# davidbau/rewriting

Measured on AMD Instinct MI355X. Metric: images/sec StyleGANv2-1024 fwd, higher is better.
Workload: dtype f32 (conv operands split into exact f16 pairs from 32x32 up, f32 accumulate); 1 GPU; stylegan2-1024 generator forward (FFHQ-1024 architecture); batch_per_gpu=64, mconv=seq, weights=synthetic seed 0, parallelism=seeds partitioned per rank, no collective, matrix_mode=split, direct_sums=auto

## Files before the change

rewriting_amd/csrc/rw_common.h:

```cpp
#pragma once
#include <hip/hip_runtime.h>
#include <stdint.h>
#include <stdlib.h>
#include "../../include/rewriting_hip.h"

#define RW_WAVE 64

#define RW_CHECK_ARG(cond) do { if (!(cond)) return RW_ERR_BAD_ARGUMENT; } while (0)
#define RW_LAUNCH_RESULT() ((int)hipGetLastError())

static inline hipStream_t rw_s(rw_stream_t s) { return (hipStream_t)s; }

static inline int64_t rw_cdiv(int64_t a, int64_t b) { return (a + b - 1) / b; }

static inline int rw_cu_count(void) {
  static int cached[64];
  int dev = 0;
  if (hipGetDevice(&dev) != hipSuccess || dev < 0 || dev >= 64) return 256;
  if (cached[dev] == 0) {
    int n = 0;
    cached[dev] = (hipDeviceGetAttribute(&n, hipDeviceAttributeMultiprocessorCount, dev) == hipSuccess && n > 0) ? n : 256;
  }
  return cached[dev];
}
// ... 104 lines not shown
    ib += g_ib + carry;
  }
};

__device__ __forceinline__ int rw_swz(int cc) { return (cc >> 1) & 3; }
__device__ __forceinline__ rw_f16x8 rw_expand(rw_f32x2 w) {
  const rw_f32x4 d = {w[0], w[1], w[0], w[1]};
  return __builtin_bit_cast(rw_f16x8, d);
}
__device__ __forceinline__ rw_f16x8 rw_pair(rw_f16x8 a, rw_f16x8 b) {
  return rw_f16x8{a[0], a[1], a[2], a[3], b[0], b[1], b[2], b[3]};
}
__device__ __forceinline__ rw_f16x8 rw_pair(rw_f32x2 a, rw_f32x2 b) {
  const rw_f32x4 d = {a[0], a[1], b[0], b[1]};
  return __builtin_bit_cast(rw_f16x8, d);
}
__device__ __forceinline__ rw_f16x8 rw_split4(float v0, float v1, float v2, float v3) {
  const rw_f16x2 h01 = __builtin_convertvector(rw_f32x2{v0, v1}, rw_f16x2);
  const rw_f16x2 h23 = __builtin_convertvector(rw_f32x2{v2, v3}, rw_f16x2);
  float r0, r1, r2, r3;
  asm("v_fma_mix_f32 %0, -%1, 1.0, %2 op_sel_hi:[1,0,0]" : "=v"(r0) : "v"(h01), "v"(v0));
  asm("v_fma_mix_f32 %0, -%1, 1.0, %2 op_sel:[1,0,0] op_sel_hi:[1,0,0]" : "=v"(r1) : "v"(h01), "v"(v1));
  asm("v_fma_mix_f32 %0, -%1, 1.0, %2 op_sel_hi:[1,0,0]" : "=v"(r2) : "v"(h23), "v"(v2));
  asm("v_fma_mix_f32 %0, -%1, 1.0, %2 op_sel:[1,0,0] op_sel_hi:[1,0,0]" : "=v"(r3) : "v"(h23), "v"(v3));
  const rw_f16x2 l01 = __builtin_convertvector(rw_f32x2{r0, r1}, rw_f16x2);
  const rw_f16x2 l23 = __builtin_convertvector(rw_f32x2{r2, r3}, rw_f16x2);
  return rw_f16x8{h01[0], h01[1], h23[0], h23[1], l01[0], l01[1], l23[0], l23[1]};
}

__device__ __forceinline__ void rw_dma_buffer_b32(unsigned lds_addr, int voffset, rw_i32x4 rsrc, int soffset) {
  asm volatile("s_mov_b32 m0, %0\n\ts_nop 0\n\tbuffer_load_dword %1, %2, %3 offen lds"
               :: "s"(lds_addr), "v"(voffset), "s"(rsrc), "s"(soffset) : "memory");
}
__device__ __forceinline__ void rw_dma_global_b32(unsigned lds_addr, const void* gptr) {
  asm volatile("s_mov_b32 m0, %0\n\ts_nop 0\n\tglobal_load_lds_dword %1, off" :: "s"(lds_addr), "v"(gptr) : "memory");
}
__device__ __forceinline__ void rw_dma_global_b128_s(unsigned lds_addr, int voffset, const void* sbase) {
  asm volatile("s_mov_b32 m0, %0\n\ts_nop 0\n\tglobal_load_lds_dwordx4 %1, %2" :: "s"(lds_addr), "v"(voffset), "s"(sbase)
               : "memory");
}

__device__ __forceinline__ void rw_lds_barrier() {
  asm volatile("" ::: "memory");
  __builtin_amdgcn_s_waitcnt(0xC07F);
  __builtin_amdgcn_s_barrier();
  asm volatile("" ::: "memory");
}

__device__ __forceinline__ __amdgpu_buffer_rsrc_t rw_image_rsrc(const float* x, int ib, int in_ch, int64_t hw) {
  return __builtin_amdgcn_make_buffer_rsrc(const_cast<float*>(x + (int64_t)ib * in_ch * hw), 0,
                                           (int)((int64_t)in_ch * hw * 4), 0x00020000);
}

static inline int64_t rw_bound_slot_capacity(int64_t n_elems) { return 2048 + n_elems / 1024 + 1; }

int rw_bound_finish(float* bound, int64_t nslots, hipStream_t stream);

__device__ __forceinline__ float rw_bound_load(const float* __restrict__ bound) {
  return rw_wave_max(bound[threadIdx.x & 63]);
}

__device__ __forceinline__ void rw_bound_store_wave(float* __restrict__ bound, float v) {
  if ((threadIdx.x & 63) == 0)
    bound[RW_BOUND_LANES + (int64_t)blockIdx.x * (blockDim.x >> 6) + (threadIdx.x >> 6)] = v;
}

// ... 72 lines not shown
```

rewriting_amd/csrc/rw_wino4.hip:

```cpp
#include "rw_common.h"

#ifndef W4_ABL
#define W4_ABL 0
#endif
#ifndef W4_SETPRIO
#define W4_SETPRIO 0
#endif

__host__ __device__ constexpr int w4_nat(int pos) { return pos < 18 ? pos : (pos < 26 ? pos + 10 : pos - 8); }

struct Wino4Problem {
  const float* x; const float* uf; float* y;
  const float* style; const float* demod; const float* noise; const float* noise_w; const float* bias;
  int batch, in_ch, out_ch, h, w;
  int groups_x, groups_y, gpw;
  float w_scale;
  int act;
  const float* rgb_weight; const float* rgb_style; const float* rgb_bias; const float* rgb_skip; float* rgb_out;
  float rgb_scale;
  const float* post;
  const float* x_amax; float* y_amax;
  float u_inv;
};

// ... 208 lines not shown
  };

  fetch(0, 0);
  uload(0, 0);
  uload(1, 1 % NC);
  stash(0);
  fetch(1 / NC, 1 % NC);
  __syncthreads();

  int c = 0, g = 0, ub = 0;
  int fg = 2 / NC, fc = 2 % NC;
  for (int v = 0; v < VT; ++v) {
    const int buf = v & 1;
    const int ub2 = ub == 0 ? 2 : ub - 1;
    if (!(W4_ABL & 2)) {
      stash(buf ^ 1);
      fetch(fg, fc);
    }
    if (!(W4_ABL & 4)) uload(ub2, c + 2 < NC ? c + 2 : c + 2 - NC);
    compute(buf, ub);
    if (c == NC - 1) {
      if (!(W4_ABL & 8) || acc[0][0] == 12345.f) group_epilogue(g);
      c = 0; ++g;
    } else { ++c; }
    if (++fc == NC) { fc = 0; ++fg; }
    ub = ub == 2 ? 0 : ub + 1;
    if (!(W4_ABL & 16)) {
      __builtin_amdgcn_s_waitcnt(0xC07F);
      __builtin_amdgcn_s_barrier();
    }
  }
}

#define W4B_PITCH 68
#ifndef W4_NTS
#define W4_NTS 0
#endif
#if W4_NTS
#define W4_STORE(ptr, val) __builtin_nontemporal_store((val), reinterpret_cast<rw_f32x4*>(ptr))
#else
#define W4_STORE(ptr, val) (*reinterpret_cast<rw_f32x4*>(ptr) = (val))
#endif
#ifndef W4C_PREFETCH
#define W4C_PREFETCH 0
#endif

__device__ __forceinline__ void w4_bt2_rows(const rw_f32x2 e0, const rw_f32x2 e2, const rw_f32x2 e4, const rw_f32x2 d1,
                                            const rw_f32x2 d2, const rw_f32x2 d3, const rw_f32x2 d4, float cA, float cB,
                                            float cC, rw_f32x2& o0, rw_f32x2& o1, rw_f32x2& o2) {
  o0 = 4.f * e0 - 5.f * e2 + e4;
  const rw_f32x2 p = d4 - cA * d2, q = cB * d3 - cC * d1;
  o1 = p + q; o2 = p - q;
}
__device__ __forceinline__ void w4_at_row(const float (&t)[6], float (&v)[4]) {
  const float s1 = t[1] + t[2], s2 = t[1] - t[2], s3 = t[3] + t[4], s4 = t[3] - t[4];
  v[0] = t[0] + s1 + s3; v[1] = s2 + 2.f * s4; v[2] = s1 + 4.f * s3; v[3] = s2 + 8.f * s4 + t[5];
}

__device__ __forceinline__ void w4_split16(float v, rw_f16x2& hh, rw_f16x2& ll) {
  if (W4_ABL & 32) { hh = __builtin_bit_cast(rw_f16x2, v); ll = hh; return; }
  hh = __builtin_convertvector(rw_f32x2{v, v}, rw_f16x2);
  float r;
  asm("v_fma_mix_f32 %0, -%1, 1.0, %2 op_sel_hi:[1,0,0]" : "=v"(r) : "v"(hh), "v"(v));
  ll = __builtin_convertvector(rw_f32x2{r, r}, rw_f16x2);
}
__device__ __forceinline__ rw_f32x4 w4_mfma16(rw_u32x2 ww, rw_f16x2 hh, rw_f16x2 ll, rw_f32x4 acc) {
  const rw_f16x4 a = __builtin_bit_cast(rw_f16x4, ww);
  const rw_f16x4 b = {hh[0], hh[1], ll[0], ll[1]};
  if (W4_ABL & 64) {
    asm volatile("" :: "v"(a), "v"(b));
    return acc;
  }
  return __builtin_amdgcn_mfma_f32_16x16x16f16(a, b, acc, 0, 0, 0);
}
__device__ __forceinline__ unsigned w4_pack16(float u) {
  const _Float16 h = (_Float16)u;
  const _Float16 l = (_Float16)(u - (float)h);
  return (unsigned)__builtin_bit_cast(unsigned short, h) | ((unsigned)__builtin_bit_cast(unsigned short, l) << 16);
}

template <int WGN, int UDEPTH, int MODE, bool STYLE, bool PS = false, bool H16 = false>
__device__ __forceinline__ void conv_wino36b_body(const Wino4Problem& p) {
  static_assert(!PS || (WGN == 2 && UDEPTH == 2), "the point split is written for the <2, 2> shape");
  constexpr bool UP = MODE == 1, RGB = MODE == 2;
  constexpr int NSZ = RGB ? 384 : (UP ? 512 : 256);
  constexpr int NST = RGB ? 3 : 16;
  constexpr int WGM = 2;
  constexpr int WAVES = WGM * WGN, THREADS = 64 * WAVES;
  constexpr int PR = 4 * WGN + 2;
  constexpr int PIECES = (PR * W4B_PITCH + 63) / 64;
  constexpr int PPW = 4 * PIECES / WAVES;
  static_assert(4 * PIECES % WAVES == 0, "patch pieces divide among the waves");
  constexpr int UPW = (9 * WGM + WAVES - 1) / WAVES;
  constexpr int PSZ = 4 * PIECES * 64;
  constexpr int USZ = WGM * 9 * 256;
  __shared__ __attribute__((aligned(16))) float Ps[3 * PSZ];
  __shared__ __attribute__((aligned(16))) float Us[UDEPTH * USZ];
  __shared__ __attribute__((aligned(16))) float Ns[WAVES * NSZ];
  __shared__ float St[512];
  __shared__ float Ct[2][16 * WGM];
  __shared__ float Cr[3][16 * WGM];
  __shared__ float Red[WAVES];

  const int tid = threadIdx.x, lane = tid & 63;
  const int wave = __builtin_amdgcn_readfirstlane(tid >> 6);
  const int wm = wave / WGN, wn = wave % WGN;
  const int lk = lane >> 4, lt = lane & 15;

  const int local = rw_xcd_remap(blockIdx.x, gridDim.x);
  const int o_tiles = p.out_ch / (16 * WGM);
  const int runs_x = p.groups_x / p.gpw;
  const int ot = local % o_tiles;
  int pg = local / o_tiles;
  const int run = pg % runs_x; pg /= runs_x;
  const int gy = pg % p.groups_y;
  const int ib = pg / p.groups_y;
  const int o0 = ot * 16 * WGM;
  const int y0 = gy * 4 * WGN, gx0 = run * p.gpw;
  const int64_t hw = (int64_t)p.h * p.w;
  const float* xb = p.x + (int64_t)ib * p.in_ch * hw;
  const int NC = p.in_ch >> 2;
  const int VT = p.gpw * NC;

  float in_scale = 1.f, out_scale = 1.f;
  if (H16) {
    float smax = p.style ? 0.f : 1.f;
    if (p.style)
      for (int i = tid; i < p.in_ch; i += THREADS) smax = fmaxf(smax, fabsf(p.style[(int64_t)ib * p.in_ch + i]));
#pragma unroll
    for (int off = 32; off; off >>= 1) smax = fmaxf(smax, __shfl_xor(smax, off));
    smax = rw_block_max<WAVES>(smax, lane, wave, Red);
    rw_split_scales<8>(rw_bound_load(p.x_amax) * smax, p.u_inv, in_scale, out_scale);
  }
  for (int i = tid; i < p.in_ch; i += THREADS) St[i] = (p.style ? p.style[(int64_t)ib * p.in_ch + i] : 1.0f) * in_scale;
  if (tid < 16 * WGM) {
    const int o = UP ? (o0 + tid) >> 2 : o0 + tid;
    const int real_ch = UP ? p.out_ch >> 2 : p.out_ch;
    Ct[0][tid] = (p.demod ? p.demod[(int64_t)ib * real_ch + o] * p.w_scale : p.w_scale) * out_scale;
    Ct[1][tid] = p.act ? p.bias[o] : 0.f;
    if (RGB) {
      const float sr = p.rgb_scale * p.rgb_style[(int64_t)ib * p.out_ch + o];
#pragma unroll
      for (int cc = 0; cc < 3; ++cc) Cr[cc][tid] = sr * p.rgb_weight[cc * p.out_ch + o];
    }
  }
  const float noise_w = p.noise ? p.noise_w[0] : 0.f;

  typedef __attribute__((address_space(3))) float* lds_f;
  const unsigned ps_base = (unsigned)(size_t)(lds_f)Ps, us_base = (unsigned)(size_t)(lds_f)Us,
                 ns_base = (unsigned)(size_t)(lds_f)Ns;
  const unsigned long long xaddr = (unsigned long long)xb;
  const rw_i32x4 xsrc = {(int)(unsigned)xaddr, (int)(unsigned)(xaddr >> 32), (int)((int64_t)p.in_ch * hw * 4),
                         0x00020000};
  const int hw4 = (int)hw * 4;
  static_assert(PIECES % PPW == 0, "a wave's pieces lie in one channel");
  const int pch = (wave * PPW) / PIECES, piece0 = (wave * PPW) % PIECES;
  int xoff[PPW];
  auto set_group = [&](int g) __attribute__((always_inline)) {
    const int x0 = (gx0 + g) * 64;
#pragma unroll
    for (int s = 0; s < PPW; ++s) {
      const int f = 64 * (piece0 + s) + lane;
      const int r = f / W4B_PITCH, c = f - r * W4B_PITCH;
      const int iy = y0 - 1 + r, ix = x0 - 1 + c;
      const bool ok = r < PR && c < W4_PC && iy >= 0 && iy < p.h && ix >= 0 && ix < p.w;
      xoff[s] = ok ? (iy * p.w + ix) * 4 : 0x7fffffff;
    }
  };
  int p_soff = 0;
  unsigned p_dst = 0;
  auto pload_begin = [&](int ring, int fg, int fc) __attribute__((always_inline)) {
    if (fc == 0) set_group(fg);
    p_soff = (4 * fc + pch) * hw4;
    p_dst = ps_base + (unsigned)((ring * PSZ + pch * (PIECES * 64) + 64 * piece0) * 4);
  };
  auto pload_piece = [&](int s) __attribute__((always_inline)) { rw_dma_buffer_b32(p_dst + 256 * s, xoff[s], xsrc, p_soff); };
  auto pload = [&](int ring, int fg, int fc) __attribute__((always_inline)) {
    pload_begin(ring, fg, fc);
#pragma unroll
    for (int s = 0; s < PPW; ++s) pload_piece(s);
  };
  const int kq_total = p.in_ch >> 2;
  const int a_lane = lane * 4;
  auto uload = [&](int ring, int kq) __attribute__((always_inline)) {
#pragma unroll
    for (int t = 0; t < UPW; ++t) {
      const int j = wave + WAVES * t;
      if (j < 9 * WGM) {
        const int ob = j / 9, q = j - 9 * ob;
        const float* src = p.uf + ((int64_t)((o0 >> 4) + ob) * kq_total + kq) * (9 * 256) + q * 256;
        rw_dma_global_b128_s(us_base + (unsigned)((ring * USZ + ob * (9 * 256) + q * 256) * 4), a_lane * 4, src);
      }
    }
  };
  auto nload = [&](int g) __attribute__((always_inline)) {
    if (UP) {
      const float* sb = p.noise + (int64_t)ib * 4 * hw + (int64_t)(2 * (y0 + 4 * wn) + 4 * wm) * (2 * p.w)
                        + (gx0 + g) * 128;
      const int vo = ((lane >> 5) * (2 * p.w) + 4 * (lane & 31)) * 4;
#pragma unroll
      for (int j = 0; j < 2; ++j)
        rw_dma_global_b128_s(ns_base + (unsigned)((wn * 1024 + (4 * wm + 2 * j) * 128) * 4), vo,
                             sb + (int64_t)(2 * j) * (2 * p.w));
      return;
    }
    const float* np = p.noise + (int64_t)ib * hw + (int64_t)(y0 + 4 * wn) * p.w + (gx0 + g) * 64 + lane;
#pragma unroll
    for (int r = 0; r < 4; ++r) rw_dma_global_b32(ns_base + (unsigned)((wave * NSZ + 64 * r) * 4), np + (int64_t)r * p.w);
  };

  rw_f32x4 acc[36];
#pragma unroll
  for (int xi = 0; xi < 36; ++xi) acc[xi] = rw_f32x4{0.f, 0.f, 0.f, 0.f};
  float ymax = 0.f;

  const int item_off = lk * (PIECES * 64) + (4 * wn) * W4B_PITCH + 4 * lt;
  auto compute = [&](int ring, int uring, int kq, auto spread_tag) __attribute__((always_inline)) {
    constexpr bool SPREAD = decltype(spread_tag)::value != 0;
    const float* base = &Us[uring * USZ + wm * (9 * 256) + a_lane];
    const float* src = &Ps[ring * PSZ + item_off];
    const float sv = St[4 * kq + lk];
    rw_f32x4 a4[3];
    a4[0] = *reinterpret_cast<const rw_f32x4*>(base);
    a4[1] = *reinterpret_cast<const rw_f32x4*>(base + 256);
    a4[2] = *reinterpret_cast<const rw_f32x4*>(base + 512);
    rw_f32x2 c2[6][3];
#pragma unroll
    for (int r = 0; r < 6; ++r) {
      const rw_f32x4 lo = *reinterpret_cast<const rw_f32x4*>(src + r * W4B_PITCH);
      if (STYLE) {
        c2[r][0] = rw_f32x2{lo[0], lo[1]} * sv;
        c2[r][1] = rw_f32x2{lo[2], lo[3]} * sv;
        c2[r][2] = *reinterpret_cast<const rw_f32x2*>(src + r * W4B_PITCH + 4) * sv;
      } else {
        c2[r][0] = rw_f32x2{lo[0], lo[1]};
        c2[r][1] = rw_f32x2{lo[2], lo[3]};
        c2[r][2] = *reinterpret_cast<const rw_f32x2*>(src + r * W4B_PITCH + 4);
      }
    }
    float d[6][6];
#pragma unroll
    for (int cp = 0; cp < 3; ++cp)
      if (!(W4_ABL & 1)) w4_bt2(c2[0][cp], c2[1][cp], c2[2][cp], c2[3][cp], c2[4][cp], c2[5][cp]);
#pragma unroll
    for (int a = 0; a < 6; ++a) {
      if (!(W4_ABL & 1)) {
        w4_bt_row(c2[a][0], c2[a][1], c2[a][2], d[a]);
      } else {
        d[a][0] = c2[a][0][0]; d[a][1] = c2[a][0][1]; d[a][2] = c2[a][1][0]; d[a][3] = c2[a][1][1];
        d[a][4] = c2[a][2][0]; d[a][5] = c2[a][2][1];
      }
    }
#if W4_SETPRIO
    __builtin_amdgcn_s_setprio(W4_SETPRIO);
#endif
#pragma unroll
    for (int q = 0; q < 9; ++q) {
      const rw_f32x4 a = a4[q % 3];
      if (q + 3 < 9) a4[q % 3] = *reinterpret_cast<const rw_f32x4*>(base + (q + 3) * 256);
      if (SPREAD && !(W4_ABL & 2)) {
        if (2 * q < PPW) pload_piece(2 * q);
        if (2 * q + 1 < PPW) pload_piece(2 * q + 1);
      }
      __builtin_amdgcn_sched_barrier(0);
#pragma unroll
      for (int e = 0; e < 4; ++e) {
        const int xi = w4_nat(4 * q + e);
        acc[xi] = __builtin_amdgcn_mfma_f32_16x16x4f32(a[e], d[xi / 6][xi % 6], acc[xi], 0, 0, 0);
      }
    }
#if W4_SETPRIO
    __builtin_amdgcn_s_setprio(0);
#endif
  };

  auto aread = [&](unsigned addr, auto pos_tag, rw_u32x2& dst) __attribute__((always_inline)) {
    constexpr int POS = decltype(pos_tag)::value;
    if (W4_ABL & 128) { dst = rw_u32x2{addr, (unsigned)POS}; return; }
    asm volatile("ds_read2st64_b32 %0, %1 offset0:%2 offset1:%2" : "=&v"(dst) : "v"(addr), "n"(POS));
  };
  auto compute16 = [&](int ring, int uring, int kq, auto spread_tag) __attribute__((always_inline)) {
    constexpr bool SPREAD = decltype(spread_tag)::value != 0;
    const unsigned ua = us_base + (unsigned)((uring * USZ + wm * (9 * 256) + lane) * 4);
    const float* src = &Ps[ring * PSZ + item_off];
    const float sv = St[4 * kq + lk];
    rw_f32x2 c2[6][3];
#pragma unroll
    for (int r = 0; r < 6; ++r) {
      const rw_f32x4 lo = *reinterpret_cast<const rw_f32x4*>(src + r * W4B_PITCH);
      c2[r][0] = rw_f32x2{lo[0], lo[1]} * sv;
      c2[r][1] = rw_f32x2{lo[2], lo[3]} * sv;
      c2[r][2] = *reinterpret_cast<const rw_f32x2*>(src + r * W4B_PITCH + 4) * sv;
    }
    rw_u32x2 aq[2][6];
    aread(ua, rw_int<0>(), aq[0][0]); aread(ua, rw_int<1>(), aq[0][1]); aread(ua, rw_int<2>(), aq[0][2]);
    aread(ua, rw_int<3>(), aq[0][3]); aread(ua, rw_int<4>(), aq[0][4]); aread(ua, rw_int<5>(), aq[0][5]);
#pragma unroll
    for (int cp = 0; cp < 3; ++cp)
      if (!(W4_ABL & 1)) w4_bt2(c2[0][cp], c2[1][cp], c2[2][cp], c2[3][cp], c2[4][cp], c2[5][cp]);
    float d[6][6];
    auto batch = [&](auto bt_tag) __attribute__((always_inline)) {
      constexpr int BT = decltype(bt_tag)::value;
      rw_u32x2 (&cur)[6] = aq[BT & 1];
      if (BT < 5) {
        rw_u32x2 (&nxt)[6] = aq[(BT + 1) & 1];
        aread(ua, rw_int<6 * BT + 6>(), nxt[0]); aread(ua, rw_int<6 * BT + 7>(), nxt[1]);
        aread(ua, rw_int<6 * BT + 8>(), nxt[2]); aread(ua, rw_int<6 * BT + 9>(), nxt[3]);
        aread(ua, rw_int<6 * BT + 10>(), nxt[4]); aread(ua, rw_int<6 * BT + 11>(), nxt[5]);
        if (!(W4_ABL & 128))
          asm volatile("s_waitcnt lgkmcnt(6)" : "+v"(cur[0]), "+v"(cur[1]), "+v"(cur[2]), "+v"(cur[3]), "+v"(cur[4]), "+v"(cur[5]) :: "memory");
      } else if (!(W4_ABL & 128)) {
        asm volatile("s_waitcnt lgkmcnt(0)" : "+v"(cur[0]), "+v"(cur[1]), "+v"(cur[2]), "+v"(cur[3]), "+v"(cur[4]), "+v"(cur[5]) :: "memory");
      }
      if (SPREAD && !(W4_ABL & 2)) {
#pragma unroll
        for (int t = 0; t < 2; ++t)
          if (2 * BT + t < PPW) pload_piece(2 * BT + t);
      }
#pragma unroll
      for (int e = 0; e < 6; ++e) {
        const int pos = 6 * BT + e;
        const int xi = w4_nat(pos);
        const int ra = xi / 6;
        if (pos == 0 || pos == 6 || pos == 12 || pos == 18 || pos == 20 || pos == 26) {
          if (!(W4_ABL & 1)) {
            w4_bt_row(c2[ra][0], c2[ra][1], c2[ra][2], d[ra]);
          } else {
            d[ra][0] = c2[ra][0][0]; d[ra][1] = c2[ra][0][1]; d[ra][2] = c2[ra][1][0]; d[ra][3] = c2[ra][1][1];
            d[ra][4] = c2[ra][2][0]; d[ra][5] = c2[ra][2][1];
          }
        }
        rw_f16x2 hh, ll;
        w4_split16(d[ra][xi % 6], hh, ll);
        acc[xi] = w4_mfma16(cur[e], hh, ll, acc[xi]);
      }
    };
    batch(rw_int<0>()); batch(rw_int<1>()); batch(rw_int<2>()); batch(rw_int<3>()); batch(rw_int<4>()); batch(rw_int<5>());
    static_assert(2 * 6 >= PPW, "two patch pieces per batch cover the wave's share");
  };

  const float ps_cA = wm ? 1.f : 4.f, ps_cB = wm ? 2.f : 1.f, ps_cC = wm ? 2.f : 4.f;
  const int ps_row = wm * W4B_PITCH;
  const int ps_quad = wm * (5 * 256), ps_half = 4 * 256 + 2 * wm;
  auto compute_ps = [&](int ring, int uring, int kq, auto spread_tag) __attribute__((always_inline)) {
    constexpr bool SPREAD = decltype(spread_tag)::value != 0;
    const float* base = &Us[uring * USZ + a_lane];
    const float* src = &Ps[ring * PSZ + item_off];
    const float sv = St[4 * kq + lk];
    rw_f32x4 a4[2][2];
    a4[0][0] = *reinterpret_cast<const rw_f32x4*>(base + ps_quad);
    a4[0][1] = *reinterpret_cast<const rw_f32x4*>(base + 9 * 256 + ps_quad);
    rw_f32x2 c2[7][3];
#pragma unroll
    for (int r = 0; r < 7; ++r) {
      const float* rp = r < 3 ? src + ps_row + 2 * r * W4B_PITCH : src + (r - 2) * W4B_PITCH;
      const rw_f32x4 lo = *reinterpret_cast<const rw_f32x4*>(rp);
      if (STYLE) {
        c2[r][0] = rw_f32x2{lo[0], lo[1]} * sv;
        c2[r][1] = rw_f32x2{lo[2], lo[3]} * sv;
        c2[r][2] = *reinterpret_cast<const rw_f32x2*>(rp + 4) * sv;
      } else {
        c2[r][0] = rw_f32x2{lo[0], lo[1]};
        c2[r][1] = rw_f32x2{lo[2], lo[3]};
        c2[r][2] = *reinterpret_cast<const rw_f32x2*>(rp + 4);
      }
    }
    rw_f32x2 hrow[3][3];
#pragma unroll
    for (int cp = 0; cp < 3; ++cp)
      w4_bt2_rows(c2[0][cp], c2[1][cp], c2[2][cp], c2[3][cp], c2[4][cp], c2[5][cp], c2[6][cp], ps_cA, ps_cB, ps_cC,
                  hrow[0][cp], hrow[1][cp], hrow[2][cp]);
    float d[3][6];
#pragma unroll
    for (int a = 0; a < 3; ++a) w4_bt_row(hrow[a][0], hrow[a][1], hrow[a][2], d[a]);
#pragma unroll
    for (int q = 0; q < 5; ++q) {
      const rw_f32x4 a0 = a4[q & 1][0], a1 = a4[q & 1][1];
      if (q + 1 < 4) {
        a4[(q + 1) & 1][0] = *reinterpret_cast<const rw_f32x4*>(base + ps_quad + (q + 1) * 256);
        a4[(q + 1) & 1][1] = *reinterpret_cast<const rw_f32x4*>(base + 9 * 256 + ps_quad + (q + 1) * 256);
      } else if (q + 1 == 4) {
        const rw_f32x2 h0 = *reinterpret_cast<const rw_f32x2*>(base + ps_half);
        const rw_f32x2 h1 = *reinterpret_cast<const rw_f32x2*>(base + 9 * 256 + ps_half);
        a4[0][0] = rw_f32x4{h0[0], h0[1], 0.f, 0.f};
        a4[0][1] = rw_f32x4{h1[0], h1[1], 0.f, 0.f};
      }
      if (SPREAD && !(W4_ABL & 2)) {
#pragma unroll
        for (int t = 0; t < 3; ++t)
          if (3 * q + t < PPW) pload_piece(3 * q + t);
      }
      __builtin_amdgcn_sched_barrier(0);
#pragma unroll
      for (int e = 0; e < (q < 4 ? 4 : 2); ++e) {
        const int le = 4 * q + e;
        acc[le] = __builtin_amdgcn_mfma_f32_16x16x4f32(a0[e], d[le / 6][le % 6], acc[le], 0, 0, 0);
        acc[18 + le] = __builtin_amdgcn_mfma_f32_16x16x4f32(a1[e], d[le / 6][le % 6], acc[18 + le], 0, 0, 0);
      }
    }
  };

  auto compute16_ps = [&](int ring, int uring, int kq, auto spread_tag) __attribute__((always_inline)) {
    constexpr bool SPREAD = decltype(spread_tag)::value != 0;
    const unsigned ua = us_base + (unsigned)((uring * USZ + lane) * 4) + (unsigned)(wm * 20 * 256);
    const unsigned ub = us_base + (unsigned)((uring * USZ + lane) * 4) + (unsigned)(wm * 2 * 256);
    const float* src = &Ps[ring * PSZ + item_off];
    const float sv = St[4 * kq + lk];
    rw_u32x2 aq[2][6];
    aread(ua, rw_int<0>(), aq[0][0]); aread(ua, rw_int<36>(), aq[0][1]); aread(ua, rw_int<1>(), aq[0][2]);
    aread(ua, rw_int<37>(), aq[0][3]); aread(ua, rw_int<2>(), aq[0][4]); aread(ua, rw_int<38>(), aq[0][5]);
    rw_f32x2 c2[7][3];
#pragma unroll
    for (int r = 0; r < 7; ++r) {
      const float* rp = r < 3 ? src + ps_row + 2 * r * W4B_PITCH : src + (r - 2) * W4B_PITCH;
      const rw_f32x4 lo = *reinterpret_cast<const rw_f32x4*>(rp);
      c2[r][0] = rw_f32x2{lo[0], lo[1]} * sv;
      c2[r][1] = rw_f32x2{lo[2], lo[3]} * sv;
      c2[r][2] = *reinterpret_cast<const rw_f32x2*>(rp + 4) * sv;
    }
    rw_f32x2 hrow[3][3];
#pragma unroll
    for (int cp = 0; cp < 3; ++cp)
      w4_bt2_rows(c2[0][cp], c2[1][cp], c2[2][cp], c2[3][cp], c2[4][cp], c2[5][cp], c2[6][cp], ps_cA, ps_cB, ps_cC,
                  hrow[0][cp], hrow[1][cp], hrow[2][cp]);
    float d[3][6];
    auto batch = [&](auto bt_tag) __attribute__((always_inline)) {
      constexpr int BT = decltype(bt_tag)::value;
      rw_u32x2 (&cur)[6] = aq[BT & 1];
      if (BT < 5) {
        rw_u32x2 (&nxt)[6] = aq[(BT + 1) & 1];
        constexpr int L0 = 3 * BT + 3, L1 = 3 * BT + 4, L2 = 3 * BT + 5;
        aread(L0 < 16 ? ua : ub, rw_int<L0>(), nxt[0]); aread(L0 < 16 ? ua : ub, rw_int<L0 + 36>(), nxt[1]);
        aread(L1 < 16 ? ua : ub, rw_int<L1>(), nxt[2]); aread(L1 < 16 ? ua : ub, rw_int<L1 + 36>(), nxt[3]);
        aread(L2 < 16 ? ua : ub, rw_int<L2>(), nxt[4]); aread(L2 < 16 ? ua : ub, rw_int<L2 + 36>(), nxt[5]);
        if (!(W4_ABL & 128))
          asm volatile("s_waitcnt lgkmcnt(6)" : "+v"(cur[0]), "+v"(cur[1]), "+v"(cur[2]), "+v"(cur[3]), "+v"(cur[4]), "+v"(cur[5]) :: "memory");
      } else if (!(W4_ABL & 128)) {
        asm volatile("s_waitcnt lgkmcnt(0)" : "+v"(cur[0]), "+v"(cur[1]), "+v"(cur[2]), "+v"(cur[3]), "+v"(cur[4]), "+v"(cur[5]) :: "memory");
      }
      if (SPREAD && !(W4_ABL & 2)) {
#pragma unroll
        for (int t = 0; t < 2; ++t)
          if (2 * BT + t < PPW) pload_piece(2 * BT + t);
      }
#pragma unroll
      for (int e = 0; e < 3; ++e) {
        const int le = 3 * BT + e;
        if (le % 6 == 0) w4_bt_row(hrow[le / 6][0], hrow[le / 6][1], hrow[le / 6][2], d[le / 6]);
        rw_f16x2 hh, ll;
        w4_split16(d[le / 6][le % 6], hh, ll);
        acc[le] = w4_mfma16(cur[2 * e], hh, ll, acc[le]);
// ... 401 lines not shown
    const int kq = (int)(rest % kqn);
    const int ob = (int)(rest / kqn);
    const int v = 16 * ob + (lane & 15), i = 4 * kq + (lane >> 4);
    const int o = v >> 2, py = (v >> 1) & 1, px = v & 1;
    const float* g = w + ((int64_t)o * in_ch + i) * 9;
    float h[9];
#pragma unroll
    for (int a = 0; a < 3; ++a)
#pragma unroll
      for (int b = 0; b < 3; ++b) {
        const int ty = 2 - 2 * a + py, tx = 2 - 2 * b + px;
        float sum = 0.f;
#pragma unroll
        for (int c = 0; c < 4; ++c)
#pragma unroll
          for (int d = 0; d < 4; ++d) {
            const int ky = ty - 1 + c, kx = tx - 1 + d;
            if (ky >= 0 && ky < 3 && kx >= 0 && kx < 3) sum += k4[(3 - c) * 4 + (3 - d)] * g[3 * ky + kx];
          }
        h[3 * a + b] = sum;
      }
    m = fmaxf(m, w4_pack_store<PASS>(h, uf + ((int64_t)ob * kqn + kq) * (9 * 256) + (PASS == 2 ? lane : lane * 4), su));
  }
  __shared__ float red[4];
  if (PASS == 1) rw_bound_store_block_256(bound, m, red);
  if (PASS == 2 && blockIdx.x == 0 && threadIdx.x < 4)
    uf[36 * total + threadIdx.x] = threadIdx.x == 0 ? 1.f / su : (threadIdx.x == 1 ? su : 0.f);
}

static bool wino4_shape_ok(int out_ch, int in_ch, int h, int w) {
  return out_ch > 0 && in_ch > 0 && out_ch % 32 == 0 && in_ch % 8 == 0 && w % 64 == 0 && h % 8 == 0;
}

extern "C" int rw_conv3x3_wino4_supported(int out_ch, int in_ch, int h, int w) {
  return wino4_shape_ok(out_ch, in_ch, h, w) ? 1 : 0;
}

extern "C" long long rw_packed_conv_weight_wino4_elems(int out_ch, int in_ch) {
  if (out_ch <= 0 || in_ch <= 0 || out_ch % 16 || in_ch % 4) return -1;
  return 36LL * out_ch * in_ch;
}

extern "C" int rw_pack_conv_weight_wino4_f32(const float* w, float* uf, int out_ch, int in_ch, rw_stream_t stream) {
  RW_CHECK_ARG(w && uf && out_ch > 0 && in_ch > 0);
  if (out_ch % 16 || in_ch % 4) return RW_ERR_UNSUPPORTED;
  const int64_t total = (int64_t)out_ch * in_ch;
  hipLaunchKernelGGL(pack_wino36_kernel<0>, dim3(rw_stream_grid(total, 256)), dim3(256), 0, rw_s(stream), w, uf, out_ch,
                     in_ch, 1.f, (float*)nullptr);
  return RW_LAUNCH_RESULT();
}

static int wino4_gpw(const Wino4Problem& p, int batch, int o_tiles) {
  return rw_groups_per_wg(p.groups_x, (int64_t)batch * p.groups_y * o_tiles, rw_env_int("RW_WINO4_GPW", 16), 1024);
}

static void wino4_fill(Wino4Problem& p, const float* x, const float* uf, float* y, int batch, int in_ch, int vch, int h,
                       int w, float w_scale, const rw_conv_epilogue* ep, float u_inv, const float* x_amax, float* y_amax) {
  p.x = x; p.uf = uf; p.y = y;
  rw_fill_epilogue(p, ep);
  p.batch = batch; p.in_ch = in_ch; p.out_ch = vch; p.h = h; p.w = w; p.w_scale = w_scale;
  p.x_amax = x_amax; p.y_amax = y_amax; p.u_inv = u_inv;
  p.groups_x = w / 64;
  p.groups_y = h / 8;
}

static int conv3x3_wino4_launch(const float* x, const float* uf, float* y, int batch, int in_ch, int out_ch, int h,
                                int w, float w_scale, const rw_conv_epilogue* ep, bool h16, float u_inv,
                                const float* x_amax, float* y_amax, rw_stream_t stream) {
  RW_CHECK_ARG(x && uf && y && batch > 0 && in_ch > 0 && out_ch > 0 && h > 0 && w > 0);
  RW_CHECK_ARG(rw_epilogue_ok(ep));
  RW_CHECK_ARG(!h16 || (x_amax && u_inv > 0.f));
  if (!wino4_shape_ok(out_ch, in_ch, h, w)) return RW_ERR_UNSUPPORTED;
  Wino4Problem p = {};
  wino4_fill(p, x, uf, y, batch, in_ch, out_ch, h, w, w_scale, ep, u_inv, x_amax, y_amax);
  const int o_tiles = out_ch / 32;
  p.gpw = wino4_gpw(p, batch, o_tiles);
  const int64_t work = (int64_t)batch * p.groups_y * (p.groups_x / p.gpw) * o_tiles;
  if (work <= 0 || work > 0x7fffffff) return RW_ERR_UNSUPPORTED;
  if (h16) {
    if (in_ch > 512) return RW_ERR_UNSUPPORTED;
    const int64_t n_out = (int64_t)batch * out_ch * h * w;
    if (rw_env_is("RW_W4H_WG8", '1') && h % 16 == 0) {
      p.groups_y = h / 16;
      p.gpw = rw_groups_per_wg(p.groups_x, 0, 4, 0);
      const int64_t work8 = (int64_t)batch * p.groups_y * (p.groups_x / p.gpw) * o_tiles;
      if (y_amax && 8 * work8 > rw_bound_slot_capacity(n_out)) return RW_ERR_UNSUPPORTED;
      hipLaunchKernelGGL(conv_wino36h_wg8_kernel, dim3((unsigned)work8), dim3(512), 0, rw_s(stream), p);
      return rw_finish_bound(y_amax, 8 * work8, stream);
    }
    if (y_amax && 4 * work > rw_bound_slot_capacity(n_out)) return RW_ERR_UNSUPPORTED;
    if (w4h_point_split(in_ch)) hipLaunchKernelGGL(conv_wino36h_ps_kernel, dim3((unsigned)work), dim3(256), 0, rw_s(stream), p);
    else hipLaunchKernelGGL(conv_wino36h_kernel, dim3((unsigned)work), dim3(256), 0, rw_s(stream), p);
    return rw_finish_bound(y_amax, 4 * work, stream);
  }
  const int version = rw_env_int("RW_WINO4_V", 3);
  if (version == 2 && h % 16 == 0 && in_ch <= 512) {
    p.groups_y = h / 16;
    p.gpw = rw_groups_per_wg(p.groups_x, (int64_t)batch * p.groups_y * o_tiles, rw_env_int("RW_WINO4_GPW", 4), 512);
    const int64_t work2 = (int64_t)batch * p.groups_y * (p.groups_x / p.gpw) * o_tiles;
    if (work2 <= 0 || work2 > 0x7fffffff) return RW_ERR_UNSUPPORTED;
    hipLaunchKernelGGL((conv_wino36b_kernel<4, 3>), dim3((unsigned)work2), dim3(512), 0, rw_s(stream), p);
    return RW_LAUNCH_RESULT();
  }
  if (version == 3 && in_ch <= 512) {
#if W4_PSPLIT
// ... 45 lines not shown
                                     float* y_amax, rw_stream_t stream) {
  return conv3x3_wino4_launch(x, uf, y, batch, in_ch, out_ch, h, w, w_scale, ep, true, u_inv, x_amax, y_amax, stream);
}

static bool up_wino4_shape_ok(int out_ch, int in_ch, int h, int w) {
  return out_ch > 0 && out_ch % 8 == 0 && in_ch >= 8 && in_ch <= 512 && in_ch % 8 == 0 && w % 64 == 0 && h % 8 == 0;
}

extern "C" int rw_conv_transpose_blur_wino4_supported(int out_ch, int in_ch, int h, int w) {
  return up_wino4_shape_ok(out_ch, in_ch, h, w) ? 1 : 0;
}

extern "C" long long rw_packed_conv_transpose_blur_wino4_elems(int out_ch, int in_ch) {
  if (out_ch <= 0 || in_ch <= 0 || out_ch % 4 || in_ch % 4) return -1;
  return 144LL * out_ch * in_ch;
}

extern "C" int rw_pack_conv_transpose_blur_weight_wino4_f32(const float* w, const float* k4, float* uf, int out_ch,
                                                            int in_ch, rw_stream_t stream) {
  RW_CHECK_ARG(w && k4 && uf && out_ch > 0 && in_ch > 0);
  if (out_ch % 4 || in_ch % 4) return RW_ERR_UNSUPPORTED;
  const int64_t total = 4LL * out_ch * in_ch;
  hipLaunchKernelGGL(pack_up_wino36_kernel<0>, dim3(rw_stream_grid(total, 256)), dim3(256), 0, rw_s(stream), w, k4, uf,
                     out_ch, in_ch, 1.f, (float*)nullptr);
  return RW_LAUNCH_RESULT();
}

static int up_wino4_launch(const float* x, const float* uf, float* y, int batch, int in_ch, int out_ch, int h, int w,
                           float w_scale, const rw_conv_epilogue* ep, const float* post_scale, bool h16, float u_inv,
                           const float* x_amax, float* y_amax, rw_stream_t stream) {
  RW_CHECK_ARG(x && uf && y && batch > 0 && in_ch > 0 && out_ch > 0 && h > 0 && w > 0);
  RW_CHECK_ARG(rw_epilogue_ok(ep));
  RW_CHECK_ARG(!h16 || (x_amax && u_inv > 0.f));
  if (!up_wino4_shape_ok(out_ch, in_ch, h, w)) return RW_ERR_UNSUPPORTED;
  Wino4Problem p = {};
  wino4_fill(p, x, uf, y, batch, in_ch, 4 * out_ch, h, w, w_scale, ep, u_inv, x_amax, y_amax);
  p.post = post_scale;
  const int o_tiles = p.out_ch / 32;
  p.gpw = wino4_gpw(p, batch, o_tiles);
  const int64_t work = (int64_t)batch * p.groups_y * (p.groups_x / p.gpw) * o_tiles;
  if (work <= 0 || work > 0x7fffffff) return RW_ERR_UNSUPPORTED;
  if (h16) {
    if (y_amax && 4 * work > rw_bound_slot_capacity((int64_t)batch * out_ch * 4 * h * w)) return RW_ERR_UNSUPPORTED;
    if (w4h_point_split(in_ch)) hipLaunchKernelGGL(conv_up_wino36h_ps_kernel, dim3((unsigned)work), dim3(256), 0, rw_s(stream), p);
    else hipLaunchKernelGGL(conv_up_wino36h_kernel, dim3((unsigned)work), dim3(256), 0, rw_s(stream), p);
    return rw_finish_bound(y_amax, 4 * work, stream);
  }
#if W4_PSPLIT
  if (w4_point_split()) {
    if (p.style) hipLaunchKernelGGL(conv_up_wino36_ps_kernel, dim3((unsigned)work), dim3(256), 0, rw_s(stream), p);
    else hipLaunchKernelGGL(conv_up_wino36_ns_ps_kernel, dim3((unsigned)work), dim3(256), 0, rw_s(stream), p);
  } else
#endif
  if (p.style) hipLaunchKernelGGL(conv_up_wino36_kernel, dim3((unsigned)work), dim3(256), 0, rw_s(stream), p);
  else hipLaunchKernelGGL(conv_up_wino36_ns_kernel, dim3((unsigned)work), dim3(256), 0, rw_s(stream), p);
  return RW_LAUNCH_RESULT();
}

extern "C" int rw_conv_transpose3x3s2_blur_wino4_f32(const float* x, const float* uf, float* y, int batch, int in_ch,
                                                     int out_ch, int h, int w, float w_scale,
                                                     const rw_conv_epilogue* ep, const float* post_scale,
                                                     rw_stream_t stream) {
  return up_wino4_launch(x, uf, y, batch, in_ch, out_ch, h, w, w_scale, ep, post_scale, false, 1.f, nullptr, nullptr, stream);
}

extern "C" long long rw_packed_conv_transpose_blur_wino4h_elems(int out_ch, int in_ch) {
  if (out_ch <= 0 || in_ch <= 0 || out_ch % 4 || in_ch % 4) return -1;
// ... 8 lines not shown
  const int grid = rw_stream_grid(total, 256);
  hipLaunchKernelGGL(pack_up_wino36_kernel<1>, dim3(grid), dim3(256), 0, rw_s(stream), w, k4, (float*)nullptr, out_ch, in_ch,
                     1.f, bound);
  return rw_finish_bound(bound, grid, stream);
}

extern "C" int rw_pack_conv_transpose_blur_weight_wino4h_f32(const float* w, const float* k4, float* uf, int out_ch,
                                                             int in_ch, float u_scale, rw_stream_t stream) {
  RW_CHECK_ARG(w && k4 && uf && out_ch > 0 && in_ch > 0 && u_scale > 0.f);
  if (out_ch % 4 || in_ch % 4) return RW_ERR_UNSUPPORTED;
  const int64_t total = 4LL * out_ch * in_ch;
  hipLaunchKernelGGL(pack_up_wino36_kernel<2>, dim3(rw_stream_grid(total, 256)), dim3(256), 0, rw_s(stream), w, k4, uf,
                     out_ch, in_ch, u_scale, (float*)nullptr);
  return RW_LAUNCH_RESULT();
}

extern "C" int rw_conv_transpose3x3s2_blur_wino4h_f32(const float* x, const float* uf, float* y, int batch, int in_ch,
                                                      int out_ch, int h, int w, float w_scale,
                                                      const rw_conv_epilogue* ep, const float* post_scale, float u_inv,
                                                      const float* x_amax, float* y_amax, rw_stream_t stream) {
  return up_wino4_launch(x, uf, y, batch, in_ch, out_ch, h, w, w_scale, ep, post_scale, true, u_inv, x_amax, y_amax, stream);
}

extern "C" int rw_conv3x3_wino4_to_rgb_supported(int out_ch, int in_ch, int h, int w) {
  return out_ch == 32 && in_ch <= 512 && wino4_shape_ok(out_ch, in_ch, h, w) ? 1 : 0;
}

static int wino4_to_rgb_launch(const float* x, const float* uf, int batch, int in_ch, int out_ch, int h, int w,
                               float w_scale, const rw_conv_epilogue* ep, const rw_rgb_epilogue* rgb, bool h16,
                               float u_inv, const float* x_amax, rw_stream_t stream) {
  RW_CHECK_ARG(x && uf && rw_rgb_ok(rgb) && batch > 0 && in_ch > 0 && out_ch > 0);
  RW_CHECK_ARG(rw_epilogue_ok(ep));
  RW_CHECK_ARG(!h16 || (x_amax && u_inv > 0.f));
  if (!rw_conv3x3_wino4_to_rgb_supported(out_ch, in_ch, h, w)) return RW_ERR_UNSUPPORTED;
  Wino4Problem p = {};
  wino4_fill(p, x, uf, nullptr, batch, in_ch, out_ch, h, w, w_scale, ep, u_inv, x_amax, nullptr);
  rw_fill_rgb(p, rgb);
  p.gpw = wino4_gpw(p, batch, 1);
  const int64_t work = (int64_t)batch * p.groups_y * (p.groups_x / p.gpw);
  if (work <= 0 || work > 0x7fffffff) return RW_ERR_UNSUPPORTED;
  if (h16) {
    if (w4h_point_split(in_ch)) hipLaunchKernelGGL(conv_wino36h_rgb_ps_kernel, dim3((unsigned)work), dim3(256), 0, rw_s(stream), p);
    else hipLaunchKernelGGL(conv_wino36h_rgb_kernel, dim3((unsigned)work), dim3(256), 0, rw_s(stream), p);
    return RW_LAUNCH_RESULT();
  }
#if W4_PSPLIT
  if (w4_point_split()) {
    if (p.style) hipLaunchKernelGGL(conv_wino36_rgb_ps_kernel, dim3((unsigned)work), dim3(256), 0, rw_s(stream), p);
    else hipLaunchKernelGGL(conv_wino36_rgb_ns_ps_kernel, dim3((unsigned)work), dim3(256), 0, rw_s(stream), p);
  } else
#endif
  if (p.style) hipLaunchKernelGGL(conv_wino36_rgb_kernel, dim3((unsigned)work), dim3(256), 0, rw_s(stream), p);
  else hipLaunchKernelGGL(conv_wino36_rgb_ns_kernel, dim3((unsigned)work), dim3(256), 0, rw_s(stream), p);
  return RW_LAUNCH_RESULT();
}

extern "C" int rw_conv3x3_wino4_to_rgb_f32(const float* x, const float* uf, int batch, int in_ch, int out_ch, int h,
                                           int w, float w_scale, const rw_conv_epilogue* ep,
                                           const rw_rgb_epilogue* rgb, rw_stream_t stream) {
  return wino4_to_rgb_launch(x, uf, batch, in_ch, out_ch, h, w, w_scale, ep, rgb, false, 1.f, nullptr, stream);
}

extern "C" int rw_conv3x3_wino4h_to_rgb_f32(const float* x, const float* uf, int batch, int in_ch, int out_ch, int h,
                                            int w, float w_scale, const rw_conv_epilogue* ep,
                                            const rw_rgb_epilogue* rgb, float u_inv, const float* x_amax,
                                            rw_stream_t stream) {
  return wino4_to_rgb_launch(x, uf, batch, in_ch, out_ch, h, w, w_scale, ep, rgb, true, u_inv, x_amax, stream);
// ... 2 lines not shown
```

Measured before the change: 1616 images/sec.

## Load Winograd input patches with 16-byte LDS DMA and realign patch rows

Input patch staging switches from per-dword buffer-to-LDS DMA to dwordx4 DMA. Each lane now fetches a 4-float aligned chunk starting at x0-4, with pitch raised to 72 and the last piece clamped to overlap. Row reads in the compute paths are rewritten to take an aligned middle vector plus two edge scalars. The Red scratch array is aliased into Ns to save LDS, and launches now reject inputs that are not 16-byte aligned. The aim is to cut the number of DMA instructions per patch, at the cost of loading some extra columns and unaligned edge LDS reads.

```diff
diff --git a/rewriting_amd/csrc/rw_common.h b/rewriting_amd/csrc/rw_common.h
--- a/rewriting_amd/csrc/rw_common.h
+++ b/rewriting_amd/csrc/rw_common.h
@@ -160,6 +160,10 @@
   asm volatile("s_mov_b32 m0, %0\n\ts_nop 0\n\tbuffer_load_dword %1, %2, %3 offen lds"
                :: "s"(lds_addr), "v"(voffset), "s"(rsrc), "s"(soffset) : "memory");
 }
+__device__ __forceinline__ void rw_dma_buffer_b128(unsigned lds_addr, int voffset, rw_i32x4 rsrc, int soffset) {
+  asm volatile("s_mov_b32 m0, %0\n\ts_nop 0\n\tbuffer_load_dwordx4 %1, %2, %3 offen lds"
+               :: "s"(lds_addr), "v"(voffset), "s"(rsrc), "s"(soffset) : "memory");
+}
 __device__ __forceinline__ void rw_dma_global_b32(unsigned lds_addr, const void* gptr) {
   asm volatile("s_mov_b32 m0, %0\n\ts_nop 0\n\tglobal_load_lds_dword %1, off" :: "s"(lds_addr), "v"(gptr) : "memory");
 }
diff --git a/rewriting_amd/csrc/rw_wino4.hip b/rewriting_amd/csrc/rw_wino4.hip
--- a/rewriting_amd/csrc/rw_wino4.hip
+++ b/rewriting_amd/csrc/rw_wino4.hip
@@ -264,7 +264,28 @@
   }
 }
 
-#define W4B_PITCH 68
+#define W4B_PITCH 72
+#ifndef W4_PAIRPAD
+#define W4_PAIRPAD 0
+#endif
+#ifndef W4_ROW3
+#define W4_ROW3 0
+#endif
+__device__ __forceinline__ void w4_row_read(const float* rp, rw_f32x2 (&c)[3], int eoff = 0) {
+  const rw_f32x4 mid = *reinterpret_cast<const rw_f32x4*>(rp + 4);
+#if W4_ROW3 == 2
+  const int edge = __float_as_int(rp[eoff]);
+  const float e0 = __int_as_float(__builtin_amdgcn_update_dpp(edge, __float_as_int(mid[3]), 0x111, 0xf, 0xf, false));
+  const float e5 = __int_as_float(__builtin_amdgcn_update_dpp(edge, __float_as_int(mid[0]), 0x101, 0xf, 0xf, false));
+#elif W4_ROW3
+  const float e0 = (*reinterpret_cast<const rw_f32x2*>(rp + 2))[1], e5 = (*reinterpret_cast<const rw_f32x2*>(rp + 8))[0];
+#else
+  const float e0 = rp[3], e5 = rp[8];
+#endif
+  c[0] = rw_f32x2{e0, mid[0]};
+  c[1] = rw_f32x2{mid[1], mid[2]};
+  c[2] = rw_f32x2{mid[3], e5};
+}
 #ifndef W4_NTS
 #define W4_NTS 0
 #endif
@@ -320,11 +341,17 @@
   constexpr int WGM = 2;
   constexpr int WAVES = WGM * WGN, THREADS = 64 * WAVES;
   constexpr int PR = 4 * WGN + 2;
-  constexpr int PIECES = (PR * W4B_PITCH + 63) / 64;
+  constexpr int IPR = W4B_PITCH / 4;
+  constexpr int ITEMS = PR * IPR;
+  constexpr int PIECES = (ITEMS + 63) / 64;
+  static_assert(ITEMS >= 64, "the last piece starts at item ITEMS - 64");
+  constexpr int CSZ = PR * W4B_PITCH;
   constexpr int PPW = 4 * PIECES / WAVES;
   static_assert(4 * PIECES % WAVES == 0, "patch pieces divide among the waves");
   constexpr int UPW = (9 * WGM + WAVES - 1) / WAVES;
-  constexpr int PSZ = 4 * PIECES * 64;
+  constexpr int CPAD = W4_PAIRPAD && !UP ? 64 - 2 * CSZ % 64 : 0;
+  constexpr int PSZ = 4 * CSZ + CPAD;
+  auto chan_off = [](int c) __attribute__((always_inline)) { return CPAD ? (c & 1) * (2 * CSZ + CPAD) + (c >> 1) * CSZ : c * CSZ; };
   constexpr int USZ = WGM * 9 * 256;
   __shared__ __attribute__((aligned(16))) float Ps[3 * PSZ];
   __shared__ __attribute__((aligned(16))) float Us[UDEPTH * USZ];
@@ -332,7 +359,9 @@
   __shared__ float St[512];
   __shared__ float Ct[2][16 * WGM];
   __shared__ float Cr[3][16 * WGM];
-  __shared__ float Red[WAVES];
+  float (&Red)[WAVES] = *reinterpret_cast<float (*)[WAVES]>(&Ns[0]);
+  static_assert(THREADS != 256 || (3 * PSZ + UDEPTH * USZ + WAVES * NSZ + 512 + 2 * 16 * WGM + (RGB ? 3 * 16 * WGM : 0)) * 4 <= 81920,
+                "LDS of a 256-thread workgroup: two must stay resident per CU");
 
   const int tid = threadIdx.x, lane = tid & 63;
   const int wave = __builtin_amdgcn_readfirstlane(tid >> 6);
@@ -387,15 +416,19 @@
   const int hw4 = (int)hw * 4;
   static_assert(PIECES % PPW == 0, "a wave's pieces lie in one channel");
   const int pch = (wave * PPW) / PIECES, piece0 = (wave * PPW) % PIECES;
+  auto piece_item0 = [&](int s) __attribute__((always_inline)) {
+    const int i0 = 64 * (piece0 + s);
+    return i0 < ITEMS - 64 ? i0 : ITEMS - 64;
+  };
   int xoff[PPW];
   auto set_group = [&](int g) __attribute__((always_inline)) {
     const int x0 = (gx0 + g) * 64;
 #pragma unroll
     for (int s = 0; s < PPW; ++s) {
-      const int f = 64 * (piece0 + s) + lane;
-      const int r = f / W4B_PITCH, c = f - r * W4B_PITCH;
-      const int iy = y0 - 1 + r, ix = x0 - 1 + c;
-      const bool ok = r < PR && c < W4_PC && iy >= 0 && iy < p.h && ix >= 0 && ix < p.w;
+      const int it = piece_item0(s) + lane;
+      const int r = it / IPR, ci = it - r * IPR;
+      const int iy = y0 - 1 + r, ix = x0 - 4 + 4 * ci;
+      const bool ok = iy >= 0 && iy < p.h && ix >= 0 && ix < p.w;
       xoff[s] = ok ? (iy * p.w + ix) * 4 : 0x7fffffff;
     }
   };
@@ -404,9 +437,11 @@
   auto pload_begin = [&](int ring, int fg, int fc) __attribute__((always_inline)) {
     if (fc == 0) set_group(fg);
     p_soff = (4 * fc + pch) * hw4;
-    p_dst = ps_base + (unsigned)((ring * PSZ + pch * (PIECES * 64) + 64 * piece0) * 4);
-  };
-  auto pload_piece = [&](int s) __attribute__((always_inline)) { rw_dma_buffer_b32(p_dst + 256 * s, xoff[s], xsrc, p_soff); };
+    p_dst = ps_base + (unsigned)((ring * PSZ + chan_off(pch)) * 4);
+  };
+  auto pload_piece = [&](int s) __attribute__((always_inline)) {
+    rw_dma_buffer_b128(p_dst + 16 * piece_item0(s), xoff[s], xsrc, p_soff);
+  };
   auto pload = [&](int ring, int fg, int fc) __attribute__((always_inline)) {
     pload_begin(ring, fg, fc);
 #pragma unroll
@@ -446,7 +481,8 @@
   for (int xi = 0; xi < 36; ++xi) acc[xi] = rw_f32x4{0.f, 0.f, 0.f, 0.f};
   float ymax = 0.f;
 
-  const int item_off = lk * (PIECES * 64) + (4 * wn) * W4B_PITCH + 4 * lt;
+  const int item_off = chan_off(lk) + (4 * wn) * W4B_PITCH + 4 * lt;
+  const int edge_off = lt == 15 ? 8 : 3 - 4 * lt;
   auto compute = [&](int ring, int uring, int kq, auto spread_tag) __attribute__((always_inline)) {
     constexpr bool SPREAD = decltype(spread_tag)::value != 0;
     const float* base = &Us[uring * USZ + wm * (9 * 256) + a_lane];
@@ -459,16 +495,8 @@
     rw_f32x2 c2[6][3];
 #pragma unroll
     for (int r = 0; r < 6; ++r) {
-      const rw_f32x4 lo = *reinterpret_cast<const rw_f32x4*>(src + r * W4B_PITCH);
-      if (STYLE) {
-        c2[r][0] = rw_f32x2{lo[0], lo[1]} * sv;
-        c2[r][1] = rw_f32x2{lo[2], lo[3]} * sv;
-        c2[r][2] = *reinterpret_cast<const rw_f32x2*>(src + r * W4B_PITCH + 4) * sv;
-      } else {
-        c2[r][0] = rw_f32x2{lo[0], lo[1]};
-        c2[r][1] = rw_f32x2{lo[2], lo[3]};
-        c2[r][2] = *reinterpret_cast<const rw_f32x2*>(src + r * W4B_PITCH + 4);
-      }
+      w4_row_read(src + r * W4B_PITCH, c2[r], edge_off);
+      if (STYLE) { c2[r][0] *= sv; c2[r][1] *= sv; c2[r][2] *= sv; }
     }
     float d[6][6];
 #pragma unroll
@@ -519,10 +547,8 @@
     rw_f32x2 c2[6][3];
 #pragma unroll
     for (int r = 0; r < 6; ++r) {
-      const rw_f32x4 lo = *reinterpret_cast<const rw_f32x4*>(src + r * W4B_PITCH);
-      c2[r][0] = rw_f32x2{lo[0], lo[1]} * sv;
-      c2[r][1] = rw_f32x2{lo[2], lo[3]} * sv;
-      c2[r][2] = *reinterpret_cast<const rw_f32x2*>(src + r * W4B_PITCH + 4) * sv;
+      w4_row_read(src + r * W4B_PITCH, c2[r], edge_off);
+      c2[r][0] *= sv; c2[r][1] *= sv; c2[r][2] *= sv;
     }
     rw_u32x2 aq[2][6];
     aread(ua, rw_int<0>(), aq[0][0]); aread(ua, rw_int<1>(), aq[0][1]); aread(ua, rw_int<2>(), aq[0][2]);
@@ -586,16 +612,8 @@
 #pragma unroll
     for (int r = 0; r < 7; ++r) {
       const float* rp = r < 3 ? src + ps_row + 2 * r * W4B_PITCH : src + (r - 2) * W4B_PITCH;
-      const rw_f32x4 lo = *reinterpret_cast<const rw_f32x4*>(rp);
-      if (STYLE) {
-        c2[r][0] = rw_f32x2{lo[0], lo[1]} * sv;
-        c2[r][1] = rw_f32x2{lo[2], lo[3]} * sv;
-        c2[r][2] = *reinterpret_cast<const rw_f32x2*>(rp + 4) * sv;
-      } else {
-        c2[r][0] = rw_f32x2{lo[0], lo[1]};
-        c2[r][1] = rw_f32x2{lo[2], lo[3]};
-        c2[r][2] = *reinterpret_cast<const rw_f32x2*>(rp + 4);
-      }
+      w4_row_read(rp, c2[r], edge_off);
+      if (STYLE) { c2[r][0] *= sv; c2[r][1] *= sv; c2[r][2] *= sv; }
     }
     rw_f32x2 hrow[3][3];
 #pragma unroll
@@ -645,10 +663,8 @@
 #pragma unroll
     for (int r = 0; r < 7; ++r) {
       const float* rp = r < 3 ? src + ps_row + 2 * r * W4B_PITCH : src + (r - 2) * W4B_PITCH;
-      const rw_f32x4 lo = *reinterpret_cast<const rw_f32x4*>(rp);
-      c2[r][0] = rw_f32x2{lo[0], lo[1]} * sv;
-      c2[r][1] = rw_f32x2{lo[2], lo[3]} * sv;
-      c2[r][2] = *reinterpret_cast<const rw_f32x2*>(rp + 4) * sv;
+      w4_row_read(rp, c2[r], edge_off);
+      c2[r][0] *= sv; c2[r][1] *= sv; c2[r][2] *= sv;
     }
     rw_f32x2 hrow[3][3];
 #pragma unroll
@@ -1116,6 +1132,8 @@
   return out_ch > 0 && in_ch > 0 && out_ch % 32 == 0 && in_ch % 8 == 0 && w % 64 == 0 && h % 8 == 0;
 }
 
+static bool w4_window_aligned(const float* x) { return ((uintptr_t)x & 15) == 0; }
+
 extern "C" int rw_conv3x3_wino4_supported(int out_ch, int in_ch, int h, int w) {
   return wino4_shape_ok(out_ch, in_ch, h, w) ? 1 : 0;
 }
@@ -1154,7 +1172,7 @@
   RW_CHECK_ARG(x && uf && y && batch > 0 && in_ch > 0 && out_ch > 0 && h > 0 && w > 0);
   RW_CHECK_ARG(rw_epilogue_ok(ep));
   RW_CHECK_ARG(!h16 || (x_amax && u_inv > 0.f));
-  if (!wino4_shape_ok(out_ch, in_ch, h, w)) return RW_ERR_UNSUPPORTED;
+  if (!wino4_shape_ok(out_ch, in_ch, h, w) || !w4_window_aligned(x)) return RW_ERR_UNSUPPORTED;
   Wino4Problem p = {};
   wino4_fill(p, x, uf, y, batch, in_ch, out_ch, h, w, w_scale, ep, u_inv, x_amax, y_amax);
   const int o_tiles = out_ch / 32;
@@ -1266,7 +1284,7 @@
   RW_CHECK_ARG(x && uf && y && batch > 0 && in_ch > 0 && out_ch > 0 && h > 0 && w > 0);
   RW_CHECK_ARG(rw_epilogue_ok(ep));
   RW_CHECK_ARG(!h16 || (x_amax && u_inv > 0.f));
-  if (!up_wino4_shape_ok(out_ch, in_ch, h, w)) return RW_ERR_UNSUPPORTED;
+  if (!up_wino4_shape_ok(out_ch, in_ch, h, w) || !w4_window_aligned(x)) return RW_ERR_UNSUPPORTED;
   Wino4Problem p = {};
   wino4_fill(p, x, uf, y, batch, in_ch, 4 * out_ch, h, w, w_scale, ep, u_inv, x_amax, y_amax);
   p.post = post_scale;
@@ -1341,7 +1359,7 @@
   RW_CHECK_ARG(x && uf && rw_rgb_ok(rgb) && batch > 0 && in_ch > 0 && out_ch > 0);
   RW_CHECK_ARG(rw_epilogue_ok(ep));
   RW_CHECK_ARG(!h16 || (x_amax && u_inv > 0.f));
-  if (!rw_conv3x3_wino4_to_rgb_supported(out_ch, in_ch, h, w)) return RW_ERR_UNSUPPORTED;
+  if (!rw_conv3x3_wino4_to_rgb_supported(out_ch, in_ch, h, w) || !w4_window_aligned(x)) return RW_ERR_UNSUPPORTED;
   Wino4Problem p = {};
   wino4_fill(p, x, uf, nullptr, batch, in_ch, out_ch, h, w, w_scale, ep, u_inv, x_amax, nullptr);
   rw_fill_rgb(p, rgb);
```

After: 1636 images/sec, median of 6. +1.2%, better.
